# guy3540/Acoustic_Locating_VQ-VAE

Hardware: AMD Instinct MI355X
Metric: spectrograms/sec (train step), speech VQ-VAE default config (higher is better)
Workload: dtype x3mx_hb

## Files before the change

### acoustic_locating_vq-vae_amd/csrc/conv1d_bf16_tile256.h

```cpp
#pragma once
#include "bf16_common.h"

namespace alvq {

constexpr int V2_M = 256, V2_R = 256, V2_K = 32;
constexpr int V2_HALF = V2_M * V2_K * 2;
constexpr int V2_CS = V2_M + 4;
constexpr int V2_EPI_LDS = 64 * V2_CS * 4;

struct FragSet {
  bf16x8_t a[8];
  bf16x8_t b[4];
};

template <int NMI, int NNI, int F16 = 0>
__device__ __forceinline__ void wave_epilogue_bf16(const ConvBArgs& a, const f32x4 (&acc)[NMI][NNI], int m0, int r0, int li,
                                                   int kq, int wm0, int wn0);

template <int OUT, int F16 = 0>
__device__ __forceinline__ void tile256_epilogue(const ConvBArgs& a, const f32x4 (&acc)[8][4], unsigned char* lds, int m0,
                                                 int r0, int wave, int tid, int li, int kq, int wm0) {
  if (OUT == 0) {
    wave_epilogue_bf16<8, 4, F16>(a, acc, m0, r0, li, kq, wm0, (wave & 3) * 64);
    return;
  }
  const float oscale = a.out_scale ? *a.out_scale : 1.f;
  float* Cs = (float*)lds;
  const int Lp1 = a.L + 1, ndata = a.B * Lp1;
  for (int slab = 0; slab < 4; ++slab) {
    if ((wave & 3) == slab) {
#pragma unroll
      for (int mi = 0; mi < 8; ++mi)
#pragma unroll
        for (int ni = 0; ni < 4; ++ni) {
          const int rl = ni * 16 + li, ml = wm0 + mi * 16 + kq * 4;
          *(f32x4*)(Cs + rl * V2_CS + ml) = acc[mi][ni];
        }
    }
    __syncthreads();
    const int rl = tid & 63, row = r0 + slab * 64 + rl;
    int b, l;
    if (row_valid(row, Lp1, ndata, &b, &l)) {
      for (int ml = tid >> 6; ml < V2_M; ml += 8) {
        const int m = m0 + ml;
        if (m >= a.M) break;
        a.y_ncl[((long)b * a.M + m) * a.L + l] = (Cs[rl * V2_CS + ml] + (a.bias ? a.bias[m] : 0.f)) * oscale;
      }
    }
    __syncthreads();
  }
}

template <int NMI, int NNI, int F16>
__device__ __forceinline__ void wave_epilogue_bf16(const ConvBArgs& a, const f32x4 (&acc)[NMI][NNI], int m0, int r0, int li,
                                                   int kq, int wm0, int wn0) {
  static_assert(NMI % 2 == 0, "fragments are swapped in pairs");
  elem_saturate<F16>();
  unsigned watch = 0;
  const int Lp1 = a.L + 1, ndata = a.B * Lp1;
  const int mb0 = m0 + wm0 + (kq & 1) * 16 + (kq >> 1) * 8;
#pragma unroll
  for (int ni = 0; ni < NNI; ++ni) {
    const int row = r0 + wn0 + ni * 16 + li;
    int b, l;
    const bool ok = row_valid(row, Lp1, ndata, &b, &l);
    const bool gaps = !__all(ok);
    const long o0 = (long)row * a.Mop + mb0;
    u16x8 s1[NMI / 2], s2[NMI / 2], mk[NMI / 2];
#pragma unroll
    for (int mp = 0; mp < NMI; mp += 2) {
      if (m0 + wm0 + mp * 16 >= a.Mop) continue;
      if (a.skip1) s1[mp / 2] = *(const u16x8*)(a.skip1 + o0 + mp * 16);
      if (a.skip2) s2[mp / 2] = *(const u16x8*)(a.skip2 + o0 + mp * 16);
      if (a.mask && !a.mask_bits) mk[mp / 2] = *(const u16x8*)(a.mask + o0 + mp * 16);
    }
    __builtin_amdgcn_sched_barrier(0);
#pragma unroll
    for (int mp = 0; mp < NMI; mp += 2) {
      if (m0 + wm0 + mp * 16 >= a.Mop) continue;
      const long o = o0 + mp * 16;
      const int mb = mb0 + mp * 16;
      float v[8];
#pragma unroll
      for (int e = 0; e < 4; ++e) {
        const u32x2 r = __builtin_amdgcn_permlane16_swap(__float_as_uint(acc[mp][ni][e]), __float_as_uint(acc[mp + 1][ni][e]),
                                                         false, false);
        v[e] = __uint_as_float(r[0]);
        v[e + 4] = __uint_as_float(r[1]);
      }
      if (a.bias) {
        if (m0 + wm0 + mp * 16 + 32 <= a.M) {
          const f32x4 b0 = *(const f32x4*)(a.bias + mb), b1 = *(const f32x4*)(a.bias + mb + 4);
#pragma unroll
          for (int e = 0; e < 4; ++e) {
            v[e] += b0[e];
            v[4 + e] += b1[e];
          }
        } else {
#pragma unroll
          for (int e = 0; e < 8; ++e) v[e] += (mb + e < a.M) ? a.bias[mb + e] : 0.f;
        }
      }
      if (a.skip1) {
#pragma unroll
        for (int e = 0; e < 8; ++e) v[e] += elem2f<F16>(s1[mp / 2][e]);
      }
      if (a.skip2) {
#pragma unroll
        for (int e = 0; e < 8; ++e) v[e] += elem2f<F16>(s2[mp / 2][e]);
      }
      if (a.relu & 1) {
#pragma unroll
        for (int e = 0; e < 8; ++e) v[e] = fmaxf(v[e], 0.f);
      }
      if (a.mask_bits) {
        const int bt = (int)a.mask_bits[o >> 3];
#pragma unroll
        for (int e = 0; e < 8; ++e) v[e] = __uint_as_float(__float_as_uint(v[e]) & (unsigned)((bt << (31 - e)) >> 31));
      } else if (a.mask) {
#pragma unroll
        for (int e = 0; e < 8; ++e) v[e] = (short)mk[mp / 2][e] > 0 ? v[e] : 0.f;
      }
      u32x4 out;
#pragma unroll
      for (int e = 0; e < 4; ++e) out[e] = elem_pk<F16>(v[2 * e], v[2 * e + 1]);
      if (gaps) {
#pragma unroll
        for (int e = 0; e < 4; ++e) out[e] = ok ? out[e] : 0u;
      }
      *(u32x4*)(a.y + o) = out;
      if (F16) {
#pragma unroll
        for (int e = 0; e < 4; ++e) fp16_watch(watch, out[e]);
      }
      if (a.y2) {
        const u16x8 ps = *(const u16x8*)(a.post + o);
        u32x4 out2;
#pragma unroll
        for (int e = 0; e < 4; ++e) out2[e] = elem_pk<F16>(v[2 * e] + elem2f<F16>(ps[2 * e]), v[2 * e + 1] + elem2f<F16>(ps[2 * e + 1]));
        if (gaps) {
#pragma unroll
          for (int e = 0; e < 4; ++e) out2[e] = ok ? out2[e] : 0u;
        }
        *(u32x4*)(a.y2 + o) = out2;
      }
      if (a.bits_out) {
        unsigned bt = 0;
#pragma unroll
        for (int e = 7; e >= 0; --e) {
          const int half = (int)((e & 1) ? (out[e >> 1] & 0xffff0000u) : (out[e >> 1] << 16));
          const int t = half > 0 ? half : 0;
          bt = __builtin_amdgcn_alignbit(bt, 0u - (unsigned)t, 31);
        }
        a.bits_out[o >> 3] = (unsigned char)bt;
      }
    }
  }
  if (F16) fp16_report(watch, a.range_flag);
}

}
```

### acoustic_locating_vq-vae_amd/csrc/conv1d_bf16_v2.hip

```cpp
#include "alvq_common.h"
#include "bf16_common.h"
#include "conv1d_bf16_tile256.h"
#include "nlc_host.h"

namespace alvq {

constexpr int V2_STAGE = 2 * V2_HALF;
constexpr int V2_NSTAGE = 4;
constexpr int V2_LDS = V2_NSTAGE * V2_STAGE;
static_assert(V2_EPI_LDS <= V2_LDS, "C slab must fit");

template <int OUT, int F16 = 0>
__global__ __launch_bounds__(512, 2) void conv1d_bf16_v2_kernel(ConvBArgs a, int KW) {
  extern __shared__ __attribute__((aligned(16))) unsigned char lds[];
  const int PAD = (KW - 1) / 2;
  const int tid = threadIdx.x, lane = tid & 63;
  const int wave = __builtin_amdgcn_readfirstlane(tid >> 6);
  const int li = lane & 15, kq = lane >> 4;
  const int wm0 = (wave >> 2) * 128, wn0 = (wave & 3) * 64;

  const int tile = xcd_remap(blockIdx.x, a.mtiles * a.rtiles);
  const int m0 = (tile % a.mtiles) * V2_M;
  const int r0 = (tile / a.mtiles) * V2_R;
  const int Cp = a.Cp;

  const int hsel = (lane >> 4) & 3;
  const int hval = (hsel == 0) ? 0 : (4 - hsel);
  const int srow = lane >> 2, sgrp = (lane & 3) ^ hval;
  const long lane_off = (long)srow * Cp + sgrp * 8;
  const u16* const wbase = a.wp + ((long)m0 + wave * 32) * Cp + lane_off;
  const u16* const xbase = a.x + ((long)r0 - PAD + wave * 32) * Cp + lane_off;
  const long tap_w = (long)a.Mp128 * Cp;

  int is_chunk = 0, is_tap = 0;
  auto issue = [&](int stage) {
    unsigned char* dst = lds + stage * V2_STAGE + wave * 2048;
    const u16* ws = wbase + is_tap * tap_w + is_chunk * V2_K;
    const u16* xs = xbase + (long)is_tap * Cp + is_chunk * V2_K;
    glds16(ws, dst);
    glds16(ws + 16L * Cp, dst + 1024);
    glds16(xs, dst + V2_HALF);
    glds16(xs + 16L * Cp, dst + V2_HALF + 1024);
    if (++is_tap == KW) {
      is_tap = 0;
      ++is_chunk;
    }
  };

  const int loff = li * 64 + ((kq ^ ((((li >> 2) & 3) == 0) ? 0 : (4 - ((li >> 2) & 3)))) << 4);
  const unsigned char* const abase = lds + wm0 * 64 + loff;
  const unsigned char* const bbase = lds + V2_HALF + wn0 * 64 + loff;
  auto rd = [&](FragSet& f, int stage) {
    const unsigned char* pa = abase + stage * V2_STAGE;
    const unsigned char* pb = bbase + stage * V2_STAGE;
#pragma unroll
    for (int mi = 0; mi < 8; ++mi) f.a[mi] = *(const bf16x8_t*)(pa + mi * 1024);
#pragma unroll
    for (int ni = 0; ni < 4; ++ni) f.b[ni] = *(const bf16x8_t*)(pb + ni * 1024);
  };

  f32x4 acc[8][4];
#pragma unroll
  for (int i = 0; i < 8; ++i)
#pragma unroll
    for (int j = 0; j < 4; ++j) acc[i][j] = f32x4{0.f, 0.f, 0.f, 0.f};
  auto mm = [&](const FragSet& f, int half) {
#pragma unroll
    for (int mi = half * 4; mi < half * 4 + 4; ++mi)
#pragma unroll
      for (int ni = 0; ni < 4; ++ni)
        acc[mi][ni] = elem_mfma16<F16>(f.a[mi], f.b[ni], acc[mi][ni]);
  };

  const int n = (Cp / V2_K) * KW;
  const bool early = wave < 4;
  FragSet f0, f1;

  issue(0);
  issue(1);
  if (n > 2) {
    issue(2);
    asm volatile("s_waitcnt vmcnt(8)" ::: "memory");
  } else {
    asm volatile("s_waitcnt vmcnt(4)" ::: "memory");
  }
  __builtin_amdgcn_s_barrier();
  rd(f0, 0);
  if (n > 2) {
    asm volatile("s_waitcnt vmcnt(4)" ::: "memory");
  } else {
    asm volatile("s_waitcnt vmcnt(0)" ::: "memory");
  }
  __builtin_amdgcn_s_barrier();

  for (int t = 0; t < n; t += 2) {
    if (t + 3 < n && early) issue((t + 3) & 3);
    mm(f0, 0);
    __builtin_amdgcn_sched_barrier(0);
    rd(f1, (t + 1) & 3);
    __builtin_amdgcn_sched_barrier(0);
    if (t + 3 < n && !early) issue((t + 3) & 3);
    mm(f0, 1);
    if (t + 3 < n) {
      asm volatile("s_waitcnt vmcnt(4)" ::: "memory");
    } else {
      asm volatile("s_waitcnt vmcnt(0)" ::: "memory");
    }
    __builtin_amdgcn_s_barrier();
    if (t + 4 < n && early) issue((t + 4) & 3);
    mm(f1, 0);
    __builtin_amdgcn_sched_barrier(0);
    if (t + 2 < n) rd(f0, (t + 2) & 3);
    __builtin_amdgcn_sched_barrier(0);
    if (t + 4 < n && !early) issue((t + 4) & 3);
    mm(f1, 1);
    if (t + 4 < n) {
      asm volatile("s_waitcnt vmcnt(4)" ::: "memory");
    } else {
      asm volatile("s_waitcnt vmcnt(0)" ::: "memory");
    }
    __builtin_amdgcn_s_barrier();
  }

  tile256_epilogue<OUT, F16>(a, acc, lds, m0, r0, wave, tid, li, kq, wm0);
}

static constexpr int wide_slot(int OUT, int F16) { return OUT * 2 + F16; }
int conv1d_bf16_v2_launch(const ConvBArgs& a_in, int KW, hipStream_t stream) {
  ConvBArgs a = a_in;
  const long rows = (long)a.rtiles * TB_R;
  a.rtiles = (int)(rows / V2_R);
  a.mtiles = (a.M + V2_M - 1) / V2_M;
  static const auto table = [] {
    KernelTable<void (*)(ConvBArgs, int), 4> t;
    for_values<0, 1>([&](auto out) { for_values<0, 1>([&](auto f16) {
      t.put(wide_slot(out, f16), conv1d_bf16_v2_kernel<out, f16>, V2_LDS);
    }); });
    return t;
  }();
  static DeviceOnce attr;
  if (attr.need()) table.raise_lds_limit();
  return table.launch(wide_slot(a.y ? 0 : 1, a.elem ? 1 : 0), dim3(a.rtiles * a.mtiles), dim3(512), stream, "alvq_conv1d_bf16(v2)", a, KW);
}

}
```

Measured before the change: 7804.

## Restructure v2 conv pipeline to 64-wide K slabs with two stages and inline DMA

```diff
diff --git a/acoustic_locating_vq-vae_amd/csrc/conv1d_bf16_tile256.h b/acoustic_locating_vq-vae_amd/csrc/conv1d_bf16_tile256.h
--- a/acoustic_locating_vq-vae_amd/csrc/conv1d_bf16_tile256.h
+++ b/acoustic_locating_vq-vae_amd/csrc/conv1d_bf16_tile256.h
@@ -3,7 +3,10 @@
 
 namespace alvq {
 
-constexpr int V2_M = 256, V2_R = 256, V2_K = 32;
+constexpr int V2_M = 256, V2_R = 256;
+constexpr int V2_KT = 64;
+constexpr int V2_SLAB = V2_M * V2_KT * 2;
+constexpr int V2_K = 32;
 constexpr int V2_HALF = V2_M * V2_K * 2;
 constexpr int V2_CS = V2_M + 4;
 constexpr int V2_EPI_LDS = 64 * V2_CS * 4;
diff --git a/acoustic_locating_vq-vae_amd/csrc/conv1d_bf16_v2.hip b/acoustic_locating_vq-vae_amd/csrc/conv1d_bf16_v2.hip
--- a/acoustic_locating_vq-vae_amd/csrc/conv1d_bf16_v2.hip
+++ b/acoustic_locating_vq-vae_amd/csrc/conv1d_bf16_v2.hip
@@ -5,8 +5,8 @@
 
 namespace alvq {
 
-constexpr int V2_STAGE = 2 * V2_HALF;
-constexpr int V2_NSTAGE = 4;
+constexpr int V2_STAGE = 2 * V2_SLAB;
+constexpr int V2_NSTAGE = 2;
 constexpr int V2_LDS = V2_NSTAGE * V2_STAGE;
 static_assert(V2_EPI_LDS <= V2_LDS, "C slab must fit");
 
@@ -24,39 +24,45 @@
   const int r0 = (tile / a.mtiles) * V2_R;
   const int Cp = a.Cp;
 
-  const int hsel = (lane >> 4) & 3;
-  const int hval = (hsel == 0) ? 0 : (4 - hsel);
-  const int srow = lane >> 2, sgrp = (lane & 3) ^ hval;
-  const long lane_off = (long)srow * Cp + sgrp * 8;
-  const u16* const wbase = a.wp + ((long)m0 + wave * 32) * Cp + lane_off;
-  const u16* const xbase = a.x + ((long)r0 - PAD + wave * 32) * Cp + lane_off;
-  const long tap_w = (long)a.Mp128 * Cp;
+  const int srow = lane >> 3, sgrp = (lane & 7) ^ srow;
+  const unsigned lane_off = (unsigned)(srow * Cp + sgrp * 8) * 2u;
+  const unsigned lds0 = (unsigned)(unsigned long)((__attribute__((address_space(3))) unsigned char*)lds);
+  auto dma = [&](const char* sbase, unsigned lds_dst) {
+    asm volatile("s_mov_b32 m0, %2\n\ts_nop 0\n\tglobal_load_lds_dwordx4 %0, %1" ::"v"(lane_off), "s"(sbase), "s"(lds_dst)
+                 : "memory");
+  };
+  const char* const wS = (const char*)(a.wp + ((long)m0 + wave * 32) * Cp);
+  const char* const xS = (const char*)(a.x + ((long)r0 - PAD + wave * 32) * Cp);
+  const long tap_w = (long)a.Mp128 * Cp * 2;
+  const long row8 = (long)Cp * 16;
+  const unsigned dW = lds0 + wave * 4096;
 
   int is_chunk = 0, is_tap = 0;
   auto issue = [&](int stage) {
-    unsigned char* dst = lds + stage * V2_STAGE + wave * 2048;
-    const u16* ws = wbase + is_tap * tap_w + is_chunk * V2_K;
-    const u16* xs = xbase + (long)is_tap * Cp + is_chunk * V2_K;
-    glds16(ws, dst);
-    glds16(ws + 16L * Cp, dst + 1024);
-    glds16(xs, dst + V2_HALF);
-    glds16(xs + 16L * Cp, dst + V2_HALF + 1024);
+    const unsigned dst = dW + stage * V2_STAGE;
+    const char* ws = wS + is_tap * tap_w + is_chunk * (V2_KT * 2);
+    const char* xs = xS + (long)is_tap * Cp * 2 + is_chunk * (V2_KT * 2);
+#pragma unroll
+    for (int q = 0; q < 4; ++q) dma(ws + q * row8, dst + q * 1024);
+#pragma unroll
+    for (int q = 0; q < 4; ++q) dma(xs + q * row8, dst + V2_SLAB + q * 1024);
     if (++is_tap == KW) {
       is_tap = 0;
       ++is_chunk;
     }
   };
 
-  const int loff = li * 64 + ((kq ^ ((((li >> 2) & 3) == 0) ? 0 : (4 - ((li >> 2) & 3)))) << 4);
-  const unsigned char* const abase = lds + wm0 * 64 + loff;
-  const unsigned char* const bbase = lds + V2_HALF + wn0 * 64 + loff;
-  auto rd = [&](FragSet& f, int stage) {
-    const unsigned char* pa = abase + stage * V2_STAGE;
-    const unsigned char* pb = bbase + stage * V2_STAGE;
+  const int loff = li * 128 + ((kq ^ (li & 7)) << 4);
+  const unsigned char* const abase = lds + wm0 * 128;
+  const unsigned char* const bbase = lds + V2_SLAB + wn0 * 128;
+  auto rd = [&](FragSet& f, int stage, int sub) {
+    const int o = stage * V2_STAGE + (loff ^ (sub * 64));
+    const unsigned char* pa = abase + o;
+    const unsigned char* pb = bbase + o;
 #pragma unroll
-    for (int mi = 0; mi < 8; ++mi) f.a[mi] = *(const bf16x8_t*)(pa + mi * 1024);
+    for (int mi = 0; mi < 8; ++mi) f.a[mi] = *(const bf16x8_t*)(pa + mi * 2048);
 #pragma unroll
-    for (int ni = 0; ni < 4; ++ni) f.b[ni] = *(const bf16x8_t*)(pb + ni * 1024);
+    for (int ni = 0; ni < 4; ++ni) f.b[ni] = *(const bf16x8_t*)(pb + ni * 2048);
   };
 
   f32x4 acc[8][4];
@@ -72,54 +78,37 @@
         acc[mi][ni] = elem_mfma16<F16>(f.a[mi], f.b[ni], acc[mi][ni]);
   };
 
-  const int n = (Cp / V2_K) * KW;
+  const int n = (Cp / V2_KT) * KW;
   const bool early = wave < 4;
   FragSet f0, f1;
 
   issue(0);
-  issue(1);
-  if (n > 2) {
-    issue(2);
+  if (n > 1) {
+    issue(1);
     asm volatile("s_waitcnt vmcnt(8)" ::: "memory");
-  } else {
-    asm volatile("s_waitcnt vmcnt(4)" ::: "memory");
-  }
-  __builtin_amdgcn_s_barrier();
-  rd(f0, 0);
-  if (n > 2) {
-    asm volatile("s_waitcnt vmcnt(4)" ::: "memory");
   } else {
     asm volatile("s_waitcnt vmcnt(0)" ::: "memory");
   }
   __builtin_amdgcn_s_barrier();
+  rd(f0, 0, 0);
 
-  for (int t = 0; t < n; t += 2) {
-    if (t + 3 < n && early) issue((t + 3) & 3);
+  for (int t = 0; t < n; ++t) {
+    const int s = t & 1;
     mm(f0, 0);
     __builtin_amdgcn_sched_barrier(0);
-    rd(f1, (t + 1) & 3);
+    rd(f1, s, 1);
     __builtin_amdgcn_sched_barrier(0);
-    if (t + 3 < n && !early) issue((t + 3) & 3);
     mm(f0, 1);
-    if (t + 3 < n) {
-      asm volatile("s_waitcnt vmcnt(4)" ::: "memory");
-    } else {
-      asm volatile("s_waitcnt vmcnt(0)" ::: "memory");
-    }
+    __builtin_amdgcn_sched_barrier(0);
+    asm volatile("s_waitcnt vmcnt(0) lgkmcnt(0)" ::: "memory");
     __builtin_amdgcn_s_barrier();
-    if (t + 4 < n && early) issue((t + 4) & 3);
+    if (t + 2 < n && early) issue(s);
     mm(f1, 0);
     __builtin_amdgcn_sched_barrier(0);
-    if (t + 2 < n) rd(f0, (t + 2) & 3);
+    if (t + 1 < n) rd(f0, s ^ 1, 0);
     __builtin_amdgcn_sched_barrier(0);
-    if (t + 4 < n && !early) issue((t + 4) & 3);
+    if (t + 2 < n && !early) issue(s);
     mm(f1, 1);
-    if (t + 4 < n) {
-      asm volatile("s_waitcnt vmcnt(4)" ::: "memory");
-    } else {
-      asm volatile("s_waitcnt vmcnt(0)" ::: "memory");
-    }
-    __builtin_amdgcn_s_barrier();
   }
 
   tile256_epilogue<OUT, F16>(a, acc, lds, m0, r0, wave, tid, li, kq, wm0);
```

Result: no change. 7816 (median of 5 runs) (+0.1%).
